# cvxpy/cvxpylayers

Hardware: AMD Instinct MI355X
Metric: forward+backward problems/sec, batch=4096 n=50 m=100 SOC (higher is better)
Workload: dtype f64; 1 GPU; config M: n=50 m=100 cones l=20 q=[10, 10, 10, 10, 10, 10, 10, 10] dense A (nnzA=5000), A,b,c batched, B=4096 per GPU, eps_abs=eps_rel=0.0001, max_iters=10000, Anderson acceleration (SCS default: acceleration_lookback=10, interval 10; engine: one-pair history); 4 distinct seeded batches resident in HBM, visited round-robin (warm-up and timed steps); step = plugin forward (layout pass + solve + sta; batch_per_gpu=4096, rotating_batches=4, parallelism=batch-shard x1

## Files before the change

### cvxpylayers_amd/csrc/ce_forward_v2.h

```cpp
#pragma once
#include "ce_common.h"
#include "ce_expcone.h"
#include "ce_wave_helpers.h"
#include "ce_psd_jacobi.h"
#include "ce_lds_fwd2.h"

#ifndef F2_MASK_MUL
#define F2_MASK_MUL 1
#endif
#if F2_MASK_MUL
#define F2_SEL(ix, expr) ((expr) * ((ix) >= 0 ? 1.0 : 0.0))
#else
#define F2_SEL(ix, expr) ((ix) >= 0 ? (expr) : 0.0)
#endif
#ifndef F2_SEG_PARTS
#define F2_SEG_PARTS 1
#endif
template <int CH, int TT, int PARTS_ = F2_SEG_PARTS, bool REDUCE = true>
__device__ __forceinline__ double seg_dot(const double (&tile)[TT], const double *vec) {
    const double2 *v2 = reinterpret_cast<const double2 *>(vec);
    double a0 = 0, a1 = 0;
    constexpr int NB = TT / 2, PARTS = NB > 8 ? PARTS_ : 1, H = (NB + PARTS - 1) / PARTS;
#pragma unroll
    for (int p = 0; p < PARTS; p++) {
#pragma unroll
        for (int k = p * H; k < (p + 1) * H && k < NB; k++) {
#ifdef F2_PROBE_HALFVEC
            const double2 v = v2[NB > 8 ? k % ((NB + 1) / 2) : k];
#else
            const double2 v = v2[k];
#endif
            a0 = fma(tile[2 * k], v.x, a0);
            a1 = fma(tile[2 * k + 1], v.y, a1);
        }
        if (p + 1 < PARTS) __builtin_amdgcn_sched_barrier(0);
    }
    if constexpr (REDUCE) return group_reduce<CH, false>(a0 + a1); else return a0 + a1;
}
template <int CH, int TT, bool REDUCE = true>
__device__ __forceinline__ double seg_dot_lds(const double *row, const double *vec) {
    const double2 *r2 = reinterpret_cast<const double2 *>(row), *v2 = reinterpret_cast<const double2 *>(vec);
    double a0 = 0, a1 = 0;
    constexpr int H = (TT / 2 + 1) / 2;
#pragma unroll
    for (int k = 0; k < H; k++) {
        const double2 r = r2[k], v = v2[k];
        a0 = fma(r.x, v.x, a0);
        a1 = fma(r.y, v.y, a1);
    }
    if constexpr (TT / 2 > 4) __builtin_amdgcn_sched_barrier(0);
#pragma unroll
    for (int k = H; k < TT / 2; k++) {
        const double2 r = r2[k], v = v2[k];
        a0 = fma(r.x, v.x, a0);
        a1 = fma(r.y, v.y, a1);
    }
    if constexpr (REDUCE) return group_reduce<CH, false>(a0 + a1); else return a0 + a1;
}

#ifndef F2_IDX_FENCE
#define F2_IDX_FENCE 8
#endif
template <int TT> constexpr int idx_stride = (TT + 3) & ~3;
template <int TT, class F>
__device__ __forceinline__ void for_each_idx(const int *__restrict__ base, int t, F &&f) {
    const int4 *ip = reinterpret_cast<const int4 *>(reinterpret_cast<const char *>(base) + (unsigned)t * (unsigned)(idx_stride<TT> * sizeof(int)));
#pragma unroll
    for (int c4 = 0; c4 < idx_stride<TT> / 4; c4++) {
        const int4 ix = ip[c4];
        if (4 * c4 + 0 < TT) f(std::integral_constant<int, 0>{}, 4 * c4 + 0, ix.x);
        if (4 * c4 + 1 < TT) f(std::integral_constant<int, 1>{}, 4 * c4 + 1, ix.y);
        if (4 * c4 + 2 < TT) f(std::integral_constant<int, 2>{}, 4 * c4 + 2, ix.z);
        if (4 * c4 + 3 < TT) f(std::integral_constant<int, 3>{}, 4 * c4 + 3, ix.w);
        if (c4 % F2_IDX_FENCE == F2_IDX_FENCE - 1) __builtin_amdgcn_sched_barrier(0);
    }
}

#ifndef F2_GATHER_CHUNK
#define F2_GATHER_CHUNK 14
#endif
template <int TT, class F>
__device__ __forceinline__ void gather_tile(const int *__restrict__ base, int t, const double *__restrict__ vals, F &&f) {
    const int4 *ip = reinterpret_cast<const int4 *>(reinterpret_cast<const char *>(base) + (unsigned)t * (unsigned)(idx_stride<TT> * sizeof(int)));
    int4 ix4[idx_stride<TT> / 4];
#pragma unroll
    for (int c4 = 0; c4 < idx_stride<TT> / 4; c4++) ix4[c4] = ip[c4];
    constexpr int CHK = F2_GATHER_CHUNK < TT ? F2_GATHER_CHUNK : TT;
#pragma unroll
    for (int k0 = 0; k0 < TT; k0 += CHK) {
        double raw[CHK];
#pragma unroll
        for (int u = 0; u < CHK; u++) {
            const int k = k0 + u < TT ? k0 + u : TT - 1;
            const int4 q = ix4[k >> 2];
            const int ix = (k & 3) == 0 ? q.x : ((k & 3) == 1 ? q.y : ((k & 3) == 2 ? q.z : q.w));
            raw[u] = vals[ix < 0 ? 0 : ix];
        }
        __builtin_amdgcn_sched_barrier(0);
#pragma unroll
        for (int u = 0; u < CHK; u++) {
            const int k = k0 + u;
            if (k < TT) {
                const int4 q = ix4[k >> 2];
                const int ix = (k & 3) == 0 ? q.x : ((k & 3) == 1 ? q.y : ((k & 3) == 2 ? q.z : q.w));
                const int msk = ~(ix >> 31);
                f(k, ix, __hiloint2double(__double2hiint(raw[u]) & msk, __double2loint(raw[u]) & msk));
            }
        }
        __builtin_amdgcn_sched_barrier(0);
    }
}

__device__ __forceinline__ void wave_lds_exchange() {
    __builtin_amdgcn_fence(__ATOMIC_RELEASE, "wavefront");
    __builtin_amdgcn_wave_barrier();
    __builtin_amdgcn_fence(__ATOMIC_ACQUIRE, "wavefront");
}

template <int CHT, int CHA, int CHG>
struct F2Co {
    int t, j1, c1, i2, c2, jg, cg;
    __device__ __forceinline__ static int thread_id(int wave) {
        int lane;
        asm volatile("v_mbcnt_lo_u32_b32 %0, -1, 0\n\tv_mbcnt_hi_u32_b32 %0, -1, %0" : "=v"(lane));
        return (wave << 6) + lane;
    }
    __device__ __forceinline__ explicit F2Co(int wave) {
        const unsigned u = (unsigned)thread_id(wave);
        t = (int)u;
        j1 = (int)(u / CHT); c1 = (int)(u % CHT); i2 = (int)(u / CHA); c2 = (int)(u % CHA); jg = (int)(u / CHG); cg = (int)(u % CHG);
    }
};

template <int K, int NWV>
__device__ __forceinline__ void block_reduce_w(double (&v)[K], unsigned maxmask, double *red, int wave) {
#pragma unroll
    for (int k = 0; k < K; k++) v[k] = ((maxmask >> k) & 1u) ? wave_reduce_dpp<true>(v[k]) : wave_reduce_dpp<false>(v[k]);
    if (__builtin_amdgcn_mbcnt_hi(~0u, __builtin_amdgcn_mbcnt_lo(~0u, 0u)) == 0) {
#pragma unroll
        for (int k = 0; k < K; k++) red[wave * K + k] = v[k];
    }
    __syncthreads();
#pragma unroll
    for (int k = 0; k < K; k++) {
        double t[NWV];
#pragma unroll
        for (int w = 0; w < NWV; w++) t[w] = red[w * K + k];
        double a = t[0];
#pragma unroll
        for (int w = 1; w < NWV; w++) a = ((maxmask >> k) & 1u) ? fmax(a, t[w]) : a + t[w];
        v[k] = a;
    }
    __syncthreads();
}

#ifdef CE_TIMING
#define F2_STAMP(i) do { __syncthreads(); if (threadIdx.x == 0) f2_tstamp[i] = __builtin_readcyclecounter(); } while (0)
#define F2_ACC(k) do { const long long t1_ = __builtin_readcyclecounter(); f2_tacc[k] += t1_ - f2_t0; f2_t0 = t1_; } while (0)
#define F2_EACC(k) do { const long long t1_ = __builtin_readcyclecounter(); f2_eacc[k] += t1_ - f2_t0; f2_t0 = t1_; } while (0)
#define F2_T0() do { f2_t0 = __builtin_readcyclecounter(); } while (0)
#else
#define F2_STAMP(i) do { } while (0)
#define F2_ACC(k) do { } while (0)
#define F2_EACC(k) do { } while (0)
#define F2_T0() do { } while (0)
#endif

#ifndef F2_WPS
#define F2_WPS 3
#endif
#ifndef F2_GJ_MFMA
#define F2_GJ_MFMA 1
#endif
template <int CHT, int T1, int CHA, int T2, int CHG, int TG, bool PSD = false, int NTH = 256, bool HASP = false, bool WL = false>
__global__ void __launch_bounds__(NTH, (NTH == 256 ? ((HASP || PSD) ? 2 : F2_WPS) : 2))
k_fwd2(DevT T, ce_settings S, const double *__restrict__ Avals, const double *__restrict__ qv, long sqk, long sqb,
       const int *__restrict__ idx_at, const int *__restrict__ idx_ar, const int *__restrict__ idx_b,
       double *__restrict__ xo, double *__restrict__ yo, double *__restrict__ so, int *__restrict__ iters_o,
       int *__restrict__ status_o, double *__restrict__ resid_o,
       const double *__restrict__ Pvals_g = nullptr, int nnzP = 0, const int *__restrict__ idx_p = nullptr,
       const int *__restrict__ row_perm = nullptr, const int *__restrict__ order = nullptr, int *__restrict__ iters2 = nullptr) {
    static_assert(!(WL && (PSD || HASP)), "wave-local cone exchange: plain cones only");
    constexpr int NT = NTH, NW = NTH / 64;
    using L = F2<CHT, T1, CHA, T2, CHG, TG, NW>;
    using Co = F2Co<CHT, CHA, CHG>;
    constexpr int MP = L::MP, NP = L::NP, VP = L::VP, OY = L::OY, OX = L::OX, OT = L::OT;
    extern __shared__ __attribute__((aligned(16))) double sm[];
    enum { SC_NB0 = 0, SC_NC0, SC_SIGMA, SC_SUMLOG, SC_RP, SC_RD, SC_GAP };
    double *const sc = sm + L::O_SC;
    double *const red = sm + L::O_RED;
    int *const socr = reinterpret_cast<int *>(sm + L::O_G);
    int *const socd = socr + MP;
    double *const Gm = sm + L::O_G + MP;

    const int tid = threadIdx.x, inst = (order && order[gridDim.x]) ? order[blockIdx.x] : blockIdx.x;
    const int wave = __builtin_amdgcn_readfirstlane(tid >> 6);
    const int n = T.n, m = T.m, l = n + m + 1, ldg = T.ldg, nq = T.nq, z = T.z;
    const int gsz = max(max(n * ldg, 4 * L::LDP), 16 * NP);
    const double *const vals = Avals + (size_t)inst * T.nnz_aug;

#ifdef CE_TIMING
    __shared__ long long f2_tstamp[24], f2_tstamp2[8];
    if (threadIdx.x < 24) f2_tstamp[threadIdx.x] = 0;
    long long f2_tacc[8] = {0, 0, 0, 0, 0, 0, 0, 0}, f2_t0 = 0;
    long long f2_eacc[8] = {0, 0, 0, 0, 0, 0, 0, 0};
#endif
    F2_STAMP(0);
    for (int i = tid; i < L::O_G; i += NT) sm[i] = 0.0;
    const double *const mtab = sm + L::O_MT;
    for (int i = tid; i < MP; i += NT) {
        int r0 = -1, d = 0;
        if (i < m) { const int c = T.rowcone[i]; if (c >= 0) { r0 = T.qoff[c]; d = T.qoff[c + 1] - r0; } }
        if constexpr (PSD) {
            for (int c = 0; c < T.ns; c++) if (i >= T.soff[c] && i < T.soff[c + 1]) { r0 = T.soff[c]; d = -(T.soff[c + 1] - r0); }
            if (i >= T.eoff && i < T.eoff + 3 * (T.nep + T.np)) { r0 = T.eoff + 3 * ((i - T.eoff) / 3); d = -3; }
        }
        socr[i] = r0; socd[i] = d;
    }
    __syncthreads();
    ce_math_table_init(sm + L::O_MT, tid);
    for (int i = tid; i < m; i += NT) { const int ix = idx_b[i]; const double v = vals[ix < 0 ? 0 : ix]; sm[L::O_BV + i] = ix >= 0 ? v : 0.0; sm[L::O_DV + i] = 1.0; }
    for (int j = tid; j < n; j += NT) { sm[L::O_CV + j] = qv[j * sqk + inst * sqb]; sm[L::O_EV + j] = 1.0; }
    __syncthreads();
    {
        double r[2] = {0, 0};
        for (int i = tid; i < m; i += NT) r[0] = fmax(r[0], fabs(sm[L::O_BV + i]));
        for (int j = tid; j < n; j += NT) r[1] = fmax(r[1], fabs(sm[L::O_CV + j]));
        block_reduce_w<2, NW>(r, 3u, red, wave);
        sc[SC_NB0] = r[0]; sc[SC_NC0] = r[1]; sc[SC_SIGMA] = 1.0; sc[9] = 0.0;
        sc[10] = sqrt((double)l); sc[11] = 1e10; sc[12] = 1e-300;
    }
    F2_STAMP(1);
    if (S.normalize) {
        const Co co(wave);
        const int j1 = co.j1, c1 = co.c1, i2 = co.i2, c2 = co.c2;
        const bool own1 = (c1 == 0) && (j1 < n), own2 = (c2 == 0) && (i2 < m);
        typedef float f2v __attribute__((ext_vector_type(2)));
        f2v atv[T1 / 2], arv[T2 / 2];
        float pf[HASP ? TG : 1];
        if constexpr (HASP) {
            const double *pv = Pvals_g + (size_t)inst * nnzP;
#pragma unroll
            for (int k = 0; k < TG; k++) { const int ix = idx_p[tid * idx_stride<TG> + k]; const double v = pv[ix < 0 ? 0 : ix]; pf[k] = ix >= 0 ? (float)v : 0.0f; }
        }
        float *const fPn = reinterpret_cast<float *>(sm + L::O_S3);
        gather_tile<T1>(idx_at, tid, vals, [&](int k, int ix, double v) { atv[k >> 1][k & 1] = ix >= 0 ? (float)(-v) : 0.0f; });
        gather_tile<T2>(idx_ar, tid, vals, [&](int k, int ix, double v) { arv[k >> 1][k & 1] = ix >= 0 ? (float)(-v) : 0.0f; });
        float *const fEt0 = reinterpret_cast<float *>(sm + L::O_S1), *const fEt1 = reinterpret_cast<float *>(sm + L::O_S2);
        float *const fDt0 = reinterpret_cast<float *>(sm + L::O_U + OY), *const fDt1 = reinterpret_cast<float *>(sm + L::O_UT + OY);
        float *const fRn = reinterpret_cast<float *>(sm + L::O_ZB + OY);
        auto clampf = [](float v) -> float { return v < (float)MIN_SCALE ? 1.0f : (v > (float)MAX_SCALE ? (float)MAX_SCALE : v); };
        double Eacc = 1.0, Dacc = 1.0;
        float ecum = 1.0f, dcum = 1.0f;
        const int blk_r0 = (i2 < m) ? socr[i2] : 0, blk_d = (i2 < m) ? abs(socd[i2]) : 0;
        F2_STAMP(14);
        F2_T0();
        for (int pass = 0; pass < NUM_RUIZ_PASSES + NUM_L2_PASSES; pass++) {
            const bool l2 = pass >= NUM_RUIZ_PASSES;
            float *const fEt = (pass & 1) ? fEt1 : fEt0;
            float *const fDt = (pass & 1) ? fDt1 : fDt0;
            float cn = 0, rn = 0;
            if (l2) {
#pragma unroll
                for (int k = 0; k < T1 / 2; k++) { cn = fmaf(atv[k].x, atv[k].x, cn); cn = fmaf(atv[k].y, atv[k].y, cn); }
#pragma unroll
                for (int k = 0; k < T2 / 2; k++) { rn = fmaf(arv[k].x, arv[k].x, rn); rn = fmaf(arv[k].y, arv[k].y, rn); }
                cn = ecum * sqrtf(group_reduce_f<CHT, false>(cn)); rn = dcum * sqrtf(group_reduce_f<CHA, false>(rn));
            } else {
                float c0 = 0, c1_ = 0, r0 = 0, r1 = 0;
#pragma unroll
                for (int k = 0; k < T1 / 2; k += 2) { c0 = fmaxf(fmaxf(c0, fabsf(atv[k].x)), fabsf(atv[k].y)); if (k + 1 < T1 / 2) c1_ = fmaxf(fmaxf(c1_, fabsf(atv[k + 1].x)), fabsf(atv[k + 1].y)); }
#pragma unroll
                for (int k = 0; k < T2 / 2; k += 2) { r0 = fmaxf(fmaxf(r0, fabsf(arv[k].x)), fabsf(arv[k].y)); if (k + 1 < T2 / 2) r1 = fmaxf(fmaxf(r1, fabsf(arv[k + 1].x)), fabsf(arv[k + 1].y)); }
                cn = ecum * group_reduce_f<CHT, true>(fmaxf(c0, c1_)); rn = dcum * group_reduce_f<CHA, true>(fmaxf(r0, r1));
            }
            if constexpr (HASP) {
                const Co cop(wave);
                float pn = 0;
                if (l2) {
#pragma unroll
                    for (int k = 0; k < TG; k++) pn = fmaf(pf[k], pf[k], pn);
                    pn = group_reduce_f<CHG, false>(pn);
                } else {
#pragma unroll
                    for (int k = 0; k < TG; k++) pn = fmaxf(pn, fabsf(pf[k]));
                    pn = group_reduce_f<CHG, true>(pn);
                }
                if (cop.cg == 0 && cop.jg < n) fPn[cop.jg] = pn;
            } else {
                if (own1) fEt[j1] = __builtin_amdgcn_rsqf(clampf(cn));
            }
            if (own2) fRn[i2] = rn;
            F2_EACC(0);
            if constexpr (WL) wave_lds_exchange(); else __syncthreads();
            if constexpr (HASP) {
                if (own1) { const float pn = fPn[j1]; fEt[j1] = __builtin_amdgcn_rsqf(clampf(l2 ? sqrtf(cn * cn + pn) : fmaxf(cn, pn))); }
            }
            constexpr int NEQ = (12 + CHA - 1) / CHA;
            float ssh = 0;
            if (blk_d > 1 && blk_d <= 12) {
                const int off = (int)__umul24((unsigned)c2, (unsigned)NEQ);
                const float *fr = fRn + blk_r0 + off;
                const int lim = blk_d - off;
                float v[NEQ];
#pragma unroll
                for (int u = 0; u < NEQ; u++) v[u] = fr[u];
#pragma unroll
                for (int u = 0; u < NEQ; u++) ssh += (u < lim) ? v[u] : 0.0f;
            }
            ssh = group_reduce_f<CHA, false>(ssh);
            if (own2) {
                float a = rn;
                const int r0 = blk_r0, d = blk_d;
                if (d > 1) {
                    float s0 = ssh, s1 = 0;
                    if (d <= 12) {
                    } else {
                        int i = 0;
                        for (; i + 1 < d; i += 2) { s0 += fRn[r0 + i]; s1 += fRn[r0 + i + 1]; }
                        if (i < d) s0 += fRn[r0 + i];
                    }
                    a = (s0 + s1) * __builtin_amdgcn_rcpf((float)d);
                }
                fDt[i2] = __builtin_amdgcn_rsqf(clampf(a));
            }
            F2_EACC(1);
            __syncthreads();
            F2_EACC(2);
            {
                const float ej = fEt[j1 < NP ? j1 : 0];
                const float di = fDt[i2 < MP ? i2 : 0];
                const f2v *d2 = reinterpret_cast<const f2v *>(fDt + T1 * c1);
                const f2v *e2 = reinterpret_cast<const f2v *>(fEt + T2 * c2);
                f2v dd[T1 / 2], ee[T2 / 2];
#pragma unroll
                for (int k = 0; k < T1 / 2; k++) dd[k] = d2[k];
#pragma unroll
                for (int k = 0; k < T2 / 2; k++) ee[k] = e2[k];
                __builtin_amdgcn_sched_barrier(0);
#pragma unroll
                for (int k = 0; k < T1 / 2; k++) atv[k] *= dd[k];
#pragma unroll
                for (int k = 0; k < T2 / 2; k++) arv[k] *= ee[k];
                ecum *= ej; dcum *= di;
                if constexpr (HASP) {
                    const Co cop(wave);
                    const float eg = fEt[cop.jg < NP ? cop.jg : 0];
                    const float2 *g2 = reinterpret_cast<const float2 *>(fEt + TG * cop.cg);
#pragma unroll
                    for (int k = 0; k < TG / 2; k++) { const float2 ee = g2[k]; pf[2 * k] *= eg * ee.x; pf[2 * k + 1] *= eg * ee.y; }
                }
                Eacc *= (double)ej; Dacc *= (double)di;
            }
            F2_EACC(3);
        }
        F2_STAMP(15);
        if (own1) sm[L::O_EV + j1] = Eacc;
        if (own2) sm[L::O_DV + i2] = Dacc;
        __syncthreads();
        double r[2] = {0, 0};
        for (int i = tid; i < m; i += NT) { const double v = sm[L::O_BV + i] * sm[L::O_DV + i]; sm[L::O_BV + i] = v; r[0] = fmax(r[0], fabs(v)); }
        for (int j = tid; j < n; j += NT) { const double v = sm[L::O_CV + j] * sm[L::O_EV + j]; sm[L::O_CV + j] = v; r[1] = fmax(r[1], fabs(v)); }
        block_reduce_w<2, NW>(r, 3u, red, wave);
        const double sigma = 1.0 / clamp_scale(fmax(r[0], r[1]));
        sc[SC_SIGMA] = sigma;
        for (int i = tid; i < m; i += NT) sm[L::O_BV + i] *= sigma;
        for (int j = tid; j < n; j += NT) sm[L::O_CV + j] *= sigma;
        for (int i = tid; i < VP; i += NT) { sm[L::O_U + i] = 0.0; sm[L::O_UT + i] = 0.0; sm[L::O_ZB + i] = 0.0; }
        for (int i = tid; i < NP; i += NT) { sm[L::O_S1 + i] = 0.0; sm[L::O_S2 + i] = 0.0; }
        __syncthreads();
    }

    F2_STAMP(2);
    double scale = S.scale, hg = 0, inv_den = 0;
    const double rho_x = S.rho_x, rtau = TAU_FACTOR, alpha = S.alpha;
    auto dyv = [&](int i) -> double { return (i < z) ? ZERO_CONE_FACTOR * scale : scale; };

    double at[T1], ar[T2];
    auto materialize_at = [&](const Co &co) {
        const double ej = sm[L::O_EV + (co.j1 < NP ? co.j1 : 0)];
        const double *dv = sm + L::O_DV + T1 * co.c1;
        gather_tile<T1>(idx_at, co.t, vals, [&](int k, int ix, double v) { at[k] = F2_SEL(ix, -v * (dv[k] * ej)); });
    };
    auto materialize_ar = [&](const Co &co) {
        const double di = sm[L::O_DV + (co.i2 < MP ? co.i2 : 0)];
        const double *evs = sm + L::O_EV + T2 * co.c2;
        gather_tile<T2>(idx_ar, co.t, vals, [&](int k, int ix, double v) { ar[k] = F2_SEL(ix, -v * (di * evs[k])); });
    };
    double gPg = 0;
    double *const PgV = Gm + gsz;
    auto materialize_p = [&](const Co &co, double (&pg)[TG]) {
        const double *pv = Pvals_g + (size_t)inst * nnzP;
        const double ej = sm[L::O_EV + (co.jg < NP ? co.jg : 0)];
        const double *evs = sm + L::O_EV + TG * co.cg;
        gather_tile<TG>(idx_p, co.t, pv, [&](int k, int ix, double v) { pg[k] = F2_SEL(ix, v * (ej * evs[k])); });
    };
    auto load_phi_tile = [&](const Co &co) {
        if (co.j1 == n) {
#pragma unroll
            for (int k = 0; k < T1; k++) at[k] = sm[L::O_PHI + OY + T1 * co.c1 + k];
        } else if (co.j1 == n + 1) {
#pragma unroll
            for (int k = 0; k < T1; k++) at[k] = (T1 * co.c1 + k < n) ? sm[L::O_PHI + OX + T1 * co.c1 + k] : 0.0;
        }
    };

    double g_scale = 0.0;
    auto refactor = [&]() {
        F2_STAMP(7);
        const Co co(wave);
        const int tid = co.t;
        const int j1 = co.j1, c1 = co.c1, i2 = co.i2, c2 = co.c2, jg = co.jg, cg = co.cg;
        const bool own1 = (c1 == 0) && (j1 < n), own2 = (c2 == 0) && (i2 < m), owng = (cg == 0) && (jg < n);
        double sreg[TG];
#pragma unroll
        for (int s = 0; s < TG; s++) sreg[s] = 0.0;
        bool fast = false, g_in_lds = false;
        if constexpr (!HASP && TG <= 14) {
            if (T.f2_neumann && g_scale > 0.0) {
                const double f = uniform_d(scale / g_scale), delta = uniform_d(rho_x * (1.0 - f) / f);
                double r[1] = {0};
                if (jg < n) {
                    const double2 *src = reinterpret_cast<const double2 *>(Gm + jg * ldg + TG * cg);
#pragma unroll
                    for (int s2 = 0; s2 < TG / 2; s2++) { const double2 v = src[s2]; r[0] = fma(v.x, v.x, fma(v.y, v.y, r[0])); }
                }
                block_reduce_w<1, NW>(r, 0u, red, wave);
                const int ex = __builtin_amdgcn_readfirstlane((__double2hiint(fabs(delta) * sqrt(r[0])) >> 20) & 0x7ff) - 1023;
                const int K = ex < -17 ? 2 : (ex < -13 ? 3 : (ex < -10 ? 4 : (ex < -7 ? 7 : 0)));
                if (K > 0) {
                    fast = true;
                    double greg[TG];
                    if (jg < n) {
                        const double2 *src = reinterpret_cast<const double2 *>(Gm + jg * ldg + TG * cg);
#pragma unroll
                        for (int s2 = 0; s2 < TG / 2; s2++) { const double2 v = src[s2]; sreg[2 * s2] = v.x; sreg[2 * s2 + 1] = v.y; }
                    }
#pragma unroll
                    for (int s = 0; s < TG; s++) greg[s] = sreg[s];
                    const int lane_base = (threadIdx.x & 63) & ~(CHG - 1);
                    for (int it = 0; it < K; it++) {
                        double zz[TG];
#pragma unroll
                        for (int s = 0; s < TG; s++) zz[s] = 0.0;
                        int goff = TG * cg;
                        asm volatile("" : "+v"(goff));
#pragma unroll
                        for (int q = 0; q < CHG; q++) {
                            const int src_lane = (lane_base + q) << 2;
#pragma unroll
                            for (int s = 0; s < TG; s++) {
                                const int kcol = TG * q + s;
                                const int lo = __builtin_amdgcn_ds_bpermute(src_lane, __double2loint(sreg[s])), hi = __builtin_amdgcn_ds_bpermute(src_lane, __double2hiint(sreg[s]));
                                const double yk = __hiloint2double(hi, lo);
                                if (kcol < n) {
                                    const double2 *gr = reinterpret_cast<const double2 *>(Gm + goff);
                                    goff += ldg;
#pragma unroll
                                    for (int s2 = 0; s2 < TG / 2; s2++) { const double2 v = gr[s2]; zz[2 * s2] = fma(yk, v.x, zz[2 * s2]); zz[2 * s2 + 1] = fma(yk, v.y, zz[2 * s2 + 1]); }
                                }
                            }
                        }
#pragma unroll
                        for (int s = 0; s < TG; s++) sreg[s] = fma(-delta, zz[s], greg[s]);
                    }
                    const double rf = 1.0 / f;
#pragma unroll
                    for (int s = 0; s < TG; s++) sreg[s] = (jg < n) ? sreg[s] * rf : 0.0;
                    __syncthreads();
                }
            }
        }
        if (!fast) {
        materialize_ar(co);
#pragma unroll
        for (int s = 0; s < TG; s++) sreg[s] = 0.0;
        {
            constexpr int NTILE = L::NTILE, LDP = L::LDP;
            typedef double v4d __attribute__((ext_vector_type(4)));
            v4d acc[NTILE];
#pragma unroll
            for (int J = 0; J < NTILE; J++) acc[J] = v4d{0.0, 0.0, 0.0, 0.0};
            const int PR = (gsz / LDP) & ~3;
            const int lane = tid & 63, lg = lane >> 4, lc = lane & 15;
            for (int p0 = 0; p0 < m; p0 += PR) {
                const int p1 = min(m, p0 + PR), rows4 = (p1 - p0 + 3) & ~3;
                if (i2 >= p0 && i2 < p1) {
                    double2 *dst = reinterpret_cast<double2 *>(Gm + (i2 - p0) * LDP + T2 * c2);
#pragma unroll
                    for (int k = 0; k < T2 / 2; k++) dst[k] = make_double2(ar[2 * k], ar[2 * k + 1]);
                }
                for (int i = tid; i < (p1 - p0) * (LDP - L::NPa); i += NT) Gm[(i / (LDP - L::NPa)) * LDP + L::NPa + i % (LDP - L::NPa)] = 0.0;
                for (int i = tid; i < (rows4 - (p1 - p0)) * LDP; i += NT) Gm[(p1 - p0) * LDP + i] = 0.0;
                __syncthreads();
                if (wave < NTILE) {
                    const double *prow = Gm + lg * LDP + lc;
                    for (int i0 = 0; i0 < rows4; i0 += 4, prow += 4 * LDP) {
                        const double a = prow[16 * wave] * dyv(p0 + i0 + lg);
#pragma unroll
                        for (int J = 0; J < NTILE; J++) acc[J] = __builtin_amdgcn_mfma_f64_16x16x4f64(a, prow[16 * J], acc[J], 0, 0, 0);
                    }
                }
                __syncthreads();
            }
            if constexpr (F2_GJ_MFMA && !HASP) {
                static_assert(8 * LDP <= 16 * NP, "two R buffers of four rows fit the exchange region");
                constexpr int MAXB = 4 * NTILE;
                const int NB = (n + 3) >> 2;
                if (wave < NTILE) {
                    static_for<NTILE>([&](auto Jc) {
                        constexpr int J = decltype(Jc)::value;
                        if (wave == J) {
#pragma unroll
                            for (int r = 0; r < 4; r++) { const int row = 16 * J + lg + 4 * r; if (lc == lg + 4 * r) acc[J][r] += (row < n ? rho_x : 1.0); }
                        }
                    });
                    if (wave == 0) {
#pragma unroll
                        for (int J = 0; J < NTILE; J++) Gm[lg * LDP + 16 * J + lc] = acc[J][0];
                    }
                }
                __syncthreads();
                F2_STAMP(8);
                F2_T0();
                static_for<MAXB>([&](auto bc) {
                    constexpr int b = decltype(bc)::value, k0 = 4 * b, wo = k0 / 16, r0 = (k0 % 16) / 4, c0 = k0 % 16;
                    constexpr int k1 = k0 + 4, wn = (k1 / 16) % NTILE, r1 = (k1 % 16) / 4;
                    if (b < NB) {
                        const double *Rb = Gm + (b & 1) * (4 * LDP);
                        double *Rn = Gm + ((b + 1) & 1) * (4 * LDP);
                        if (wave < NTILE) {
                            double Bop[NTILE], Cop[4], a[4][4];
#pragma unroll
                            for (int J = 0; J < NTILE; J++) Bop[J] = Rb[lg * LDP + 16 * J + lc];
                            {
                                int coff = 16 * wave + lc;
                                asm volatile("" : "+v"(coff));
#pragma unroll
                                for (int pq = 0; pq < 4; pq++) Cop[pq] = Rb[pq * LDP + coff];
                            }
#pragma unroll
                            for (int q = 0; q < 4; q++) {
                                const double2 v0 = *reinterpret_cast<const double2 *>(Rb + q * LDP + k0), v1 = *reinterpret_cast<const double2 *>(Rb + q * LDP + k0 + 2);
                                a[q][0] = v0.x; a[q][1] = v0.y; a[q][2] = v1.x; a[q][3] = v1.y;
                            }
                            __builtin_amdgcn_sched_barrier(0);
                            double e[4];
#pragma unroll
                            for (int k = 0; k < 4; k++) e[k] = (lg == k) ? 1.0 : 0.0;
                            double pinv[4];
#pragma unroll
                            for (int k = 0; k < 4; k++) {
                                const double pv = a[k][k];
                                double pi_ = __builtin_amdgcn_rcp(pv);
                                pi_ = fma(fma(-pv, pi_, 1.0), pi_, pi_);
                                pi_ = fma(fma(-pv, pi_, 1.0), pi_, pi_);
                                pinv[k] = pi_;
#pragma unroll
                                for (int i = k + 1; i < 4; i++) {
                                    const double lm = a[i][k] * pi_;
#pragma unroll
                                    for (int j = k + 1; j < 4; j++) a[i][j] = fma(-lm, a[k][j], a[i][j]);
                                    e[i] = fma(-lm, e[k], e[i]);
                                }
                            }
                            double xs[4];
                            xs[3] = e[3] * pinv[3];
                            xs[2] = fma(-a[2][3], xs[3], e[2]) * pinv[2];
                            xs[1] = fma(-a[1][3], xs[3], fma(-a[1][2], xs[2], e[1])) * pinv[1];
                            xs[0] = fma(-a[0][3], xs[3], fma(-a[0][2], xs[2], fma(-a[0][1], xs[1], e[0]))) * pinv[0];
                            F2_EACC(4);
                            double wsel = -(Cop[0] * xs[0] + Cop[1] * xs[1] + Cop[2] * xs[2] + Cop[3] * xs[3]);
                            const int mr = lc - c0;
                            const bool kcol = mr >= 0 && mr < 4;
                            const double nk = kcol ? 0.0 : 1.0;
                            if (wave == wo) {
                                double psel = 0.0;
#pragma unroll
                                for (int k = 0; k < 4; k++) psel = fma(xs[k], (mr == k) ? 1.0 : 0.0, psel);
                                wsel = fma(wsel, nk, psel);
#pragma unroll
                                for (int J = 0; J < NTILE; J++) acc[J][r0] = 0.0;
                            }
#pragma unroll
                            for (int r = 0; r < 4; r++) acc[wo][r] *= nk;
                            Bop[wo] = fma(Bop[wo], nk, (kcol && mr == lg) ? -1.0 : 0.0);
                            F2_EACC(5);
#pragma unroll
                            for (int J = 0; J < NTILE; J++) acc[J] = __builtin_amdgcn_mfma_f64_16x16x4f64(wsel, Bop[J], acc[J], 0, 0, 0);
                            F2_EACC(6);
                            if (b + 1 < NB && wave == wn) {
#pragma unroll
                                for (int J = 0; J < NTILE; J++) Rn[lg * LDP + 16 * J + lc] = acc[J][r1];
                            }
                        }
                        __syncthreads();
                        F2_EACC(7);
                    }
                });
                F2_STAMP(9);
                if (wave < NTILE) {
#pragma unroll
                    for (int J = 0; J < NTILE; J++)
#pragma unroll
                        for (int r = 0; r < 4; r++) {
                            const int row = 16 * wave + lg + 4 * r, col = 16 * J + lc;
                            if (row < n && col < L::NPg) Gm[row * ldg + col] = 0.0 - acc[J][r];
                        }
                }
                g_in_lds = true;
            } else {
                if (wave < NTILE) {
#pragma unroll
                    for (int J = 0; J < NTILE; J++)
#pragma unroll
                        for (int r = 0; r < 4; r++) {
                            const int row = 16 * wave + lg + 4 * r, col = 16 * J + lc;
                            if (row < n && col < L::NPg) Gm[row * ldg + col] = acc[J][r] + (row == col ? rho_x : 0.0);
                        }
                }
                __syncthreads();
                if (jg < n) {
                    const double2 *src = reinterpret_cast<const double2 *>(Gm + jg * ldg + TG * cg);
#pragma unroll
                    for (int s = 0; s < TG / 2; s++) { const double2 v = src[s]; sreg[2 * s] = v.x; sreg[2 * s + 1] = v.y; }
                }
                __syncthreads();
                if constexpr (HASP) {
                    double pg[TG];
                    materialize_p(co, pg);
#pragma unroll
                    for (int s = 0; s < TG; s++) if (jg < n) sreg[s] += pg[s];
                }
            }
        }
        if (!g_in_lds) {
        F2_STAMP(8);
        constexpr int NBLK = (TG + 3) / 4;
        auto rbuf = [&](int b) -> double * { return Gm + b * (8 * NP); };
        auto cbuf = [&](int b) -> double * { return Gm + b * (8 * NP) + 4 * NP; };
        auto publish = [&](auto blk_c, int cgn, int bufn) {
            constexpr int kk0 = 4 * decltype(blk_c)::value;
            const int k0 = TG * cgn + kk0;
            if (jg < n && cg == cgn) {
                double2 *dst = reinterpret_cast<double2 *>(cbuf(bufn) + 4 * jg);
                dst[0] = make_double2(sreg[kk0], sreg[kk0 + 1]);
                if constexpr (kk0 + 3 < TG) dst[1] = make_double2(sreg[kk0 + 2], sreg[kk0 + 3]);
            }
            if (jg >= k0 && jg < k0 + (TG - kk0 < 4 ? TG - kk0 : 4) && jg < n) {
                double2 *dst = reinterpret_cast<double2 *>(rbuf(bufn) + (jg - k0) * NP + TG * cg);
#pragma unroll
                for (int s = 0; s < TG / 2; s++) dst[s] = make_double2(sreg[2 * s], sreg[2 * s + 1]);
            }
        };
        for (int i = tid; i < 16 * NP; i += NT) Gm[i] = 0.0;
        __syncthreads();
        int cnt = 0;
        publish(std::integral_constant<int, 0>{}, 0, 0);
        __syncthreads();
        F2_T0();
        static_for<NBLK>([&](auto blk_c) {
            constexpr int blk = decltype(blk_c)::value, kk0 = 4 * blk;
            constexpr int NBS = (TG - kk0) < 4 ? (TG - kk0) : 4;
            const int nv = (kk0 < n) ? (n - 1 - kk0) / TG + 1 : 0;
            const int nvn = (kk0 + 4 < TG && kk0 + 4 < n) ? 1 : 0;
            for (int cgk = 0; cgk < nv; cgk++) {
                const int k0 = TG * cgk + kk0, buf = cnt & 1;
                const int nbv = min(NBS, n - k0);
                const double *rb = rbuf(buf), *cb = cbuf(buf);
                if (jg < n) {
                    double a[4][4];
#pragma unroll
                    for (int q = 0; q < 4; q++) {
                        const double2 v0 = *reinterpret_cast<const double2 *>(rb + q * NP + k0), v1 = *reinterpret_cast<const double2 *>(rb + q * NP + k0 + 2);
                        a[q][0] = v0.x; a[q][1] = v0.y; a[q][2] = v1.x; a[q][3] = v1.y;
                    }
                    if (nbv < 4) {
#pragma unroll
                        for (int q = 0; q < 4; q++)
#pragma unroll
                            for (int q2 = 0; q2 < 4; q2++) if (!(q < nbv && q2 < nbv)) a[q][q2] = (q == q2 ? 1.0 : 0.0);
                    }
                    bool bad = false;
#pragma unroll
                    for (int p = 0; p < 4; p++) {
                        const double pv = a[p][p];
                        bad = bad || !(pv > 0);
                        double pinv = __builtin_amdgcn_rcp(pv);
                        pinv = fma(fma(-pv, pinv, 1.0), pinv, pinv);
                        pinv = fma(fma(-pv, pinv, 1.0), pinv, pinv);
#pragma unroll
                        for (int j = 0; j < 4; j++) if (j != p) a[p][j] *= pinv;
#pragma unroll
                        for (int i = 0; i < 4; i++) if (i != p) {
                            const double f = a[i][p];
#pragma unroll
                            for (int j = 0; j < 4; j++) if (j != p) a[i][j] = fma(-f, a[p][j], a[i][j]);
                            a[i][p] = -f * pinv;
                        }
                        a[p][p] = pinv;
                    }
                    F2_EACC(4);
                    if constexpr (HASP) { if (bad && jg == k0 && cg == 0) sc[7] = 1.0; }
                    const double2 c01 = reinterpret_cast<const double2 *>(cb + 4 * jg)[0];
                    double2 c23 = make_double2(0.0, 0.0);
                    if constexpr (NBS > 2) c23 = reinterpret_cast<const double2 *>(cb + 4 * jg)[1];
                    const int qrow = jg - k0;
                    const bool prow_thread = (qrow >= 0 && qrow < NBS);
                    double w[4];
#pragma unroll
                    for (int q = 0; q < 4; q++) {
                        const double wc = -(c01.x * a[0][q] + c01.y * a[1][q] + c23.x * a[2][q] + c23.y * a[3][q]);
                        const double wp = qrow == 0 ? a[0][q] : (qrow == 1 ? a[1][q] : (qrow == 2 ? a[2][q] : a[3][q]));
                        w[q] = prow_thread ? wp : wc;
                    }
                    F2_EACC(5);
                    const double2 *r0 = reinterpret_cast<const double2 *>(rb + TG * cg), *r1 = reinterpret_cast<const double2 *>(rb + NP + TG * cg),
                                  *r2 = reinterpret_cast<const double2 *>(rb + 2 * NP + TG * cg), *r3 = reinterpret_cast<const double2 *>(rb + 3 * NP + TG * cg);
#pragma unroll
                    for (int s2 = 0; s2 < TG / 2; s2++) {
                        const double2 v0 = r0[s2], v1 = r1[s2], v2 = r2[s2], v3 = r3[s2];
                        const double bx = prow_thread ? 0.0 : sreg[2 * s2], by = prow_thread ? 0.0 : sreg[2 * s2 + 1];
                        sreg[2 * s2] = fma(w[3], v3.x, fma(w[2], v2.x, fma(w[1], v1.x, fma(w[0], v0.x, bx))));
                        sreg[2 * s2 + 1] = fma(w[3], v3.y, fma(w[2], v2.y, fma(w[1], v1.y, fma(w[0], v0.y, by))));
                    }
                    if (cg == cgk) {
#pragma unroll
                        for (int q = 0; q < NBS; q++) sreg[kk0 + q] = w[q];
                    }
                }
                F2_EACC(6);
                if (cgk + 1 < nv) publish(std::integral_constant<int, blk>{}, cgk + 1, buf ^ 1);
                else if (nvn) publish(std::integral_constant<int, (blk + 1 < NBLK ? blk + 1 : blk)>{}, 0, buf ^ 1);
                cnt++;
                __syncthreads();
                F2_EACC(7);
            }
        });
        F2_STAMP(9);
        }
        }
        g_scale = uniform_d(scale);
        if constexpr (HASP) { if (sc[7] != 0.0) return; }
        if (!g_in_lds && jg < n) {
            double2 *dst = reinterpret_cast<double2 *>(Gm + jg * ldg + TG * cg);
#pragma unroll
            for (int s = 0; s < TG / 2; s++) dst[s] = make_double2(sreg[2 * s], sreg[2 * s + 1]);
        }
        for (int i = tid; i < NP; i += NT) { sm[L::O_S1 + i] = 0.0; sm[L::O_S2 + i] = 0.0; sm[L::O_S3 + i] = 0.0; sm[L::O_S4 + i] = 0.0; }
        for (int i = tid; i < m; i += NT) sm[L::O_ZB + OY + i] = dyv(i) * sm[L::O_BV + i];
        __syncthreads();
        materialize_at(co);
        {
            const double a = seg_dot<CHT, T1>(at, sm + L::O_ZB + OY + T1 * c1);
            if (own1) { const double cj = sm[L::O_CV + j1]; sm[L::O_S1 + j1] = cj - a; sm[L::O_S2 + j1] = cj + a; }
        }
        __syncthreads();
        F2_STAMP(11);
        {
            const double *grow = Gm + (jg < n ? jg : 0) * ldg + TG * cg;
            const double gx = seg_dot_lds<CHG, TG>(grow, sm + L::O_S1 + TG * cg), gk = seg_dot_lds<CHG, TG>(grow, sm + L::O_S2 + TG * cg);
            if (owng) { sm[L::O_GV + OX + jg] = gx; sm[L::O_PX + jg] = gk; }
        }
        __syncthreads();
        F2_STAMP(12);
        if constexpr (HASP) {
            double pg[TG];
            materialize_p(co, pg);
            const double a = seg_dot<CHG, TG>(pg, sm + L::O_GV + OX + TG * cg);
            if (owng) PgV[jg] = a;
            __syncthreads();
            double rg[1] = {tid < n ? sm[L::O_GV + OX + tid] * PgV[tid] : 0.0};
            block_reduce_w<1, NW>(rg, 0u, red, wave);
            gPg = uniform_d(rg[0]);
        }
        materialize_ar(co);
        double r[1] = {0};
        {
            const double agx = seg_dot<CHA, T2>(ar, sm + L::O_GV + OX + T2 * c2);
            __builtin_amdgcn_sched_barrier(0);
            const double agk = seg_dot<CHA, T2>(ar, sm + L::O_PX + T2 * c2);
            __builtin_amdgcn_sched_barrier(0);
            if (own2) {
                const double bi = sm[L::O_BV + i2];
                const double gy = dyv(i2) * (agx + bi);
                sm[L::O_GV + OY + i2] = gy; r[0] += bi * gy;
                sm[L::O_PHI + OY + i2] = bi - agk;
            }
            if (tid < n) { r[0] += sm[L::O_CV + tid] * sm[L::O_GV + OX + tid]; sm[L::O_PHI + OX + tid] = rho_x * sm[L::O_PX + tid]; }
        }
        F2_STAMP(13);
        block_reduce_w<1, NW>(r, 0u, red, wave);
        hg = uniform_d(r[0]);
        inv_den = uniform_d(1.0 / (rtau + hg));
        load_phi_tile(co);
        for (int i = tid; i < NP; i += NT) { sm[L::O_S1 + i] = 0.0; sm[L::O_S2 + i] = 0.0; sm[L::O_PX + i] = 0.0; }
        for (int i = tid; i < m; i += NT) sm[L::O_ZB + OY + i] = 0.0;
        __syncthreads();
        F2_STAMP(10);
    };

    if (threadIdx.x == 0) sm[L::O_W + OT] = 1.0;
    if (S.warm_start) {
        const double sg = sc[SC_SIGMA];
        const int inst_ = inst;
        double wx = 0, wy = 0; bool bad = false;
        const int e = threadIdx.x;
        if (e < n) { wx = sg * xo[(size_t)inst_ * n + e] / sm[L::O_EV + e]; bad = !(fabs(wx) < 1e300); }
        for (int i = e; i < m; i += NT) {
            const double dvi = sm[L::O_DV + i];
            const int io = WL ? row_perm[i] : i;
            const double v = sg * yo[(size_t)inst_ * m + io] / dvi + sg * dvi * so[(size_t)inst_ * m + io] * dyv(i);
            bad = bad || !(fabs(v) < 1e300);
        }
        double rb[1] = {bad ? 1.0 : 0.0};
        block_reduce_w<1, NW>(rb, 1u, red, wave);
        if (rb[0] == 0.0) {
            if (e < n) sm[L::O_W + OX + e] = wx;
            for (int i = e; i < m; i += NT) {
                const double dvi = sm[L::O_DV + i];
                const int io = WL ? row_perm[i] : i;
                sm[L::O_W + OY + i] = sg * yo[(size_t)inst_ * m + io] / dvi + sg * dvi * so[(size_t)inst_ * m + io] * dyv(i);
            }
        }
    }
    __syncthreads();

    int status = 0, iter = 0, last_scale_iter = 0, n_log = 0;
    int aa_ph = 0, chk_ph = 0;
    auto next_iter = [&]() { iter++; aa_ph = (aa_ph + 1 >= S.acceleration_interval) ? 0 : aa_ph + 1; chk_ph = (chk_ph + 1 == CONVERGED_INTERVAL) ? 0 : chk_ph + 1; };
    bool aa_on = S.acceleration_lookback > 0;
    const int aa_int = S.acceleration_interval;
    double *const aaWP = Gm + gsz + (PSD ? ((T.ns > 0 ? 2 * T.maxs * T.maxs + 2 * T.maxs + 8 : 0) + T.nep + T.np) : 0) + (HASP ? NP : 0);
    double *const aaXP = aaWP + VP, *const aaFP = aaXP + VP, *const aaFS = aaFP + VP, *const aaXS = aaFS + VP;
    int aa_iter = 0; bool aa_pending = false, aa_stale = false;
    const bool big_soc = T.maxq > SOC_SMALL;
    bool resume = false;

    auto project_e = [&](int e, int ve) -> double {
        double ue = sm[L::O_ZB + ve];
        const int soc_d = (e < m) ? socd[e] : 0;
        if (soc_d > 1 && !big_soc) {
            const int soc_r0 = socr[e];
            const double *zc = sm + L::O_ZB + OY + soc_r0;
            const double t0 = zc[0];
            double q0 = 0, q1 = 0;
            if (soc_d <= 13) {
                double zv[12];
#pragma unroll
                for (int u = 0; u < 12; u++) zv[u] = zc[1 + u];
#pragma unroll
                for (int u = 0; u < 12; u += 2) {
                    const double z0 = (1 + u < soc_d) ? zv[u] : 0.0, z1 = (2 + u < soc_d) ? zv[u + 1] : 0.0;
                    q0 = fma(z0, z0, q0); q1 = fma(z1, z1, q1);
                }
            } else {
                for (int k = 1; k < soc_d; k += 4) {
                    const double z0 = zc[k], z1 = (k + 1 < soc_d) ? zc[k + 1] : 0.0, z2 = (k + 2 < soc_d) ? zc[k + 2] : 0.0, z3 = (k + 3 < soc_d) ? zc[k + 3] : 0.0;
                    q0 = fma(z0, z0, q0); q1 = fma(z1, z1, q1); q0 = fma(z2, z2, q0); q1 = fma(z3, z3, q1);
                }
            }
            const double q = q0 + q1;
            double nz = 0, rinv = 0;
            if (q > 0) sqrt_rsqrt(q, nz, rinv);
            if (nz <= t0) {  }
            else if (nz <= -t0) ue = 0.0;
            else { const double c0 = 0.5 * (t0 + nz); ue = (e == soc_r0) ? c0 : ue * (c0 * rinv); }
        } else if (soc_d == 1) ue = fmax(ue, 0.0);
        return ue;
    };
    auto slot_of = [&](int e) -> int { return (e < m) ? OY + e : (e < m + n ? OX + (e - m) : OT); };

    if constexpr (PSD) {
        double *expR0 = Gm + gsz + (T.ns > 0 ? 2 * T.maxs * T.maxs + 2 * T.maxs + 8 : 0);
        for (int c = tid; c < T.nep + T.np; c += NT) expR0[c] = 0.0;
    }
    for (bool done = false; !done;) {
    refactor();
    if constexpr (HASP) { if (sc[7] != 0.0) { status = -4; break; } }
    F2_STAMP(3);
    if (resume) {
        const int e = Co::thread_id(wave);
        if (e < l) { const int ve = slot_of(e); sm[L::O_W + ve] += alpha * (sm[L::O_U + ve] - sm[L::O_UT + ve]); }
        __syncthreads();
        resume = false; next_iter();
    }
    for (;;) {
        if (iter >= S.max_iters) { done = true; break; }
        const Co co(wave);
        const int j1 = co.j1, c1 = co.c1, i2 = co.i2, c2 = co.c2, jg = co.jg, cg = co.cg;
        const bool own1 = (c1 == 0) && (j1 < n), own2 = (c2 == 0) && (i2 < m), owng = (cg == 0) && (jg < n);
        const int e = co.t;
        const int ve = slot_of(e);
        const bool ev = e < l;
        const bool check = chk_ph == 0;
        const bool last = iter + 1 >= S.max_iters;
        F2_ACC(6);
        if (aa_on) {
            if (aa_pending) {
                const double dd = ev ? aaWP[ve] - sm[L::O_W + ve] : 0.0;
                double r[1] = {dd * dd};
                block_reduce_w<1, NW>(r, 0u, red, wave);
                if (!(uniform_d(r[0]) <= sc[8])) {
                    if (ev) { sm[L::O_W + ve] = aaFS[ve]; aaWP[ve] = aaXS[ve]; }
                    aa_iter = 0;
                    if (Co::thread_id(wave) == 0) sc[9] += 1.0;
                    __syncthreads();
                    if (uniform_d(sc[9]) >= AA_MAX_REJECT) aa_on = false;
                }
                aa_pending = false;
            }
            if (aa_on && iter > 0 && aa_ph == 0 && !aa_stale) {
                const double xv = ev ? aaWP[ve] : 0.0, fv = ev ? sm[L::O_W + ve] : 0.0, gv = xv - fv;
                if (aa_iter > 0) {
                    const double xp = ev ? aaXP[ve] : 0.0, fp = ev ? aaFP[ve] : 0.0;
                    const double sv = xv - xp, yv = gv - (xp - fp), dv = fv - fp;
                    double r[5] = {sv * sv, yv * yv, sv * yv, sv * gv, gv * gv};
                    block_reduce_w<5, NW>(r, 0u, red, wave);
                    double s01 = 0, ri01 = 0;
                    { const double q01 = r[0] * r[1]; if (q01 > 0) sqrt_rsqrt(q01, s01, ri01); }
                    const double mm = uniform_d(r[2] + 1e-8 * s01);
                    double mi = __builtin_amdgcn_rcp(mm);
                    mi = fma(fma(-mm, mi, 1.0), mi, mi);
                    mi = fma(fma(-mm, mi, 1.0), mi, mi);
                    const double gam = uniform_d(r[3] * mi);
                    if (ev) { aaXP[ve] = xv; aaFP[ve] = fv; }
                    int o11 = 11; asm volatile("" : "+s"(o11));
                    if (fabs(mm) > sc[o11 + 1]  && fabs(gam) < sc[o11] ) {
                        if (ev) { aaFS[ve] = fv; aaXS[ve] = xv; sm[L::O_W + ve] = fv - gam * dv; }
                        if (Co::thread_id(wave) == 0) sc[8] = r[4];
                        aa_pending = true;
                    } else aa_iter = 0;
                } else if (ev) { aaXP[ve] = xv; aaFP[ve] = fv; }
                aa_iter++;
                __syncthreads();
            }
        }
        if (check && iter > 0) {
            const double we = ev ? sm[L::O_W + ve] : 0.0;
            double r[1] = {we * we};
            block_reduce_w<1, NW>(r, 0u, red, wave);
            const double nw = uniform_d(sqrt(r[0]));
            if (nw > 0 && ev) {
                int o10 = 10; asm volatile("" : "+s"(o10));
                const double fsc = sc[o10] / nw;
                sm[L::O_W + ve] = we * fsc;
                if (aa_on) {
                    aaXP[ve] *= fsc; aaFP[ve] *= fsc; aaFS[ve] *= fsc; aaXS[ve] *= fsc;
                    if (e == 0) sc[8] *= fsc * fsc;
                }
            }
            __syncthreads();
        }
        if (aa_on && (aa_pending || aa_ph + 1 == aa_int)) { aa_stale = false; if (ev) aaWP[ve] = sm[L::O_W + ve]; }
        F2_ACC(0);
        {
            const double *wvec = sm + L::O_W + ((j1 == n + 1 && T1 * c1 < n) ? OX : OY) + T1 * c1;
            const double a = seg_dot<CHT, T1>(at, wvec);
            if (own1) sm[L::O_TV + j1] = rho_x * sm[L::O_W + OX + j1] - a;
            else if (c1 == 0 && j1 <= n + 1) sm[L::O_WP + (j1 - n)] = a;
        }
        F2_ACC(1);
        __syncthreads();
        F2_ACC(2);
        {
            const double a = seg_dot_lds<CHG, TG>(Gm + __mul24(jg < n ? jg : 0, ldg) + TG * cg, sm + L::O_TV + TG * cg);
            if (owng) sm[L::O_PX + jg] = a;
            if (WL && Co::thread_id(wave) == 0) sm[L::O_WP + 2] = sm[L::O_W + OT];
        }
        F2_ACC(3);
        __syncthreads();
        F2_ACC(2);
        if constexpr (WL) {
            const int ee = OY + i2;
            const bool upd = !check && !last;
            double we = 0, gve = 0;
            int cd = 0, soc_r0 = 0;
            if (own2) { we = sm[L::O_W + ee]; gve = sm[L::O_GV + ee]; }
            if (i2 < m) { cd = socd[i2]; soc_r0 = socr[i2]; }
            const double wp0 = sm[L::O_WP], wp1 = sm[L::O_WP + 1], wp2 = sm[L::O_WP + 2];
            const double q = seg_dot<CHA, T2>(ar, sm + L::O_PX + T2 * c2);
            __builtin_amdgcn_sched_barrier(0);
            const double tau_t = (rtau * wp2 + wp0 + wp1) * inv_den;
            double ute = 0, ze = 0;
            if (own2) {
                const double py = we + dyv(i2) * q;
                ute = py - tau_t * gve;
                ze = 2 * ute - we;
                if (cd == 1 && ze < 0) ze = 0;
                sm[L::O_UT + ee] = ute; sm[L::O_ZB + ee] = ze;
            }
            F2_ACC(4);
            wave_lds_exchange();
            constexpr int NE = (12 + CHA - 1) / CHA;
            double qsh = 0;
            if (cd > 1 && cd <= 13) {
                const int off = (int)__umul24((unsigned)c2, (unsigned)NE);
                const double *zc = sm + L::O_ZB + OY + soc_r0 + 1 + off;
                const int lim = cd - 1 - off;
                double zv[NE];
#pragma unroll
                for (int u = 0; u < NE; u++) zv[u] = zc[u];
                double q0 = 0, q1 = 0;
#pragma unroll
                for (int u = 0; u < NE; u++) {
                    const double zz = (u < lim) ? zv[u] : 0.0;
                    if (u & 1) q1 = fma(zz, zz, q1); else q0 = fma(zz, zz, q0);
                }
                qsh = q0 + q1;
            }
            qsh = group_reduce<CHA, false>(qsh);
            if (own2) {
                double ue = ze;
                if (cd > 1) {
                    const double *zc = sm + L::O_ZB + OY + soc_r0;
                    const double t0 = zc[0];
                    double q0 = qsh, q1 = 0;
                    if (cd <= 13) {
                    } else {
                        for (int k = 1; k < cd; k += 4) {
                            const double z0 = zc[k], z1 = (k + 1 < cd) ? zc[k + 1] : 0.0, z2 = (k + 2 < cd) ? zc[k + 2] : 0.0, z3 = (k + 3 < cd) ? zc[k + 3] : 0.0;
                            q0 = fma(z0, z0, q0); q1 = fma(z1, z1, q1); q0 = fma(z2, z2, q0); q1 = fma(z3, z3, q1);
                        }
                    }
                    const double qq = q0 + q1;
                    double nz = 0, rinv = 0;
                    if (qq > 0) sqrt_rsqrt(qq, nz, rinv);
                    if (nz <= t0) {  }
                    else if (nz <= -t0) ue = 0.0;
                    else { const double c0 = 0.5 * (t0 + nz); ue = (i2 == soc_r0) ? c0 : ue * (c0 * rinv); }
                }
                sm[L::O_U + ee] = ue;
                if (upd) sm[L::O_W + ee] = we + alpha * (ue - ute);
            }
            if (e < n) {
                const int ex = OX + e;
                const double wx = sm[L::O_W + ex];
                const double utx = sm[L::O_PX + e] - tau_t * sm[L::O_GV + ex];
                const double ux = 2 * utx - wx;
                sm[L::O_UT + ex] = utx; sm[L::O_U + ex] = ux;
                if (upd) sm[L::O_W + ex] = wx + alpha * (ux - utx);
            }
            if (e == NT - 1) {
                const double wt = sm[L::O_W + OT];
                const double ut = fmax(0.0, 2 * tau_t - wt);
                sm[L::O_UT + OT] = tau_t; sm[L::O_U + OT] = ut;
                if (upd) sm[L::O_W + OT] = wt + alpha * (ut - tau_t);
            }
            F2_ACC(5);
            __syncthreads();
            F2_ACC(2);
            if (upd) { next_iter(); continue; }
        } else {
        {
            const double wt0 = sm[L::O_W + OT], wp0 = sm[L::O_WP], wp1 = sm[L::O_WP + 1];
            const double q = seg_dot<CHA, T2>(ar, sm + L::O_PX + T2 * c2);
            __builtin_amdgcn_sched_barrier(0);
            double tau_t = (rtau * wt0 + wp0 + wp1) * inv_den;
            if constexpr (HASP) {
                double r3[3] = {0, 0, 0};
                if (own2) { const double py = sm[L::O_W + OY + i2] + dyv(i2) * q; r3[0] = q * py; }
                if (e < n) { const double px = sm[L::O_PX + e]; r3[1] = px * (sm[L::O_W + OX + e] - px); r3[2] = px * PgV[e]; }
                block_reduce_w<3, NW>(r3, 0u, red, wave);
                const double pPp = rho_x * r3[1] - r3[0];
                const double qa = rtau + hg - gPg, qb = -(rtau * sm[L::O_W + OT] + sm[L::O_WP] + sm[L::O_WP + 1]) + 2 * r3[2];
                tau_t = uniform_d((-qb + sqrt(fmax(qb * qb + 4 * qa * fmax(pPp, 0.0), 0.0))) / (2 * qa));
            }
            if (own2) {
                const int ee = OY + i2;
                const double we = sm[L::O_W + ee];
                const double py = we + dyv(i2) * q;
                const double ute = py - tau_t * sm[L::O_GV + ee];
                double ze = 2 * ute - we;
                if (i2 >= z && i2 < z + T.l && ze < 0) ze = 0;
                sm[L::O_UT + ee] = ute; sm[L::O_ZB + ee] = ze;
            }
            if (e < n) {
                const int ee = OX + e;
                const double ute = sm[L::O_PX + e] - tau_t * sm[L::O_GV + ee];
// ... 185 lines not shown
```

Before: 1.979 million problems/s.

## Build transposed A tile via LDS transpose and keep ar registers across phases

In the normalize phase, the transposed tile (atv) is no longer gathered a second time from global memory. It is built by writing the already-gathered row tile (arv) into LDS as floats and reading it back column-wise. A KEEP_AR mode also keeps the equilibrated ar registers alive from the factorization phase, so the later materialize_ar gather is skipped when the non-fast path ran. The gather-chunk size for these one-shot gathers is raised to the full tile. The intent is to cut redundant global gathers at the cost of extra LDS traffic, barriers and register pressure.

New measurement: 1.969 million problems/s (median of 2 runs). No clear change (-0.5%).

```diff
diff --git a/cvxpylayers_amd/csrc/ce_forward_v2.h b/cvxpylayers_amd/csrc/ce_forward_v2.h
--- a/cvxpylayers_amd/csrc/ce_forward_v2.h
+++ b/cvxpylayers_amd/csrc/ce_forward_v2.h
@@ -79,13 +79,15 @@
 #ifndef F2_GATHER_CHUNK
 #define F2_GATHER_CHUNK 14
 #endif
-template <int TT, class F>
-__device__ __forceinline__ void gather_tile(const int *__restrict__ base, int t, const double *__restrict__ vals, F &&f) {
+template <int TT>
+__device__ __forceinline__ void load_idx_row(const int *__restrict__ base, int t, int4 (&ix4)[idx_stride<TT> / 4]) {
     const int4 *ip = reinterpret_cast<const int4 *>(reinterpret_cast<const char *>(base) + (unsigned)t * (unsigned)(idx_stride<TT> * sizeof(int)));
-    int4 ix4[idx_stride<TT> / 4];
 #pragma unroll
     for (int c4 = 0; c4 < idx_stride<TT> / 4; c4++) ix4[c4] = ip[c4];
-    constexpr int CHK = F2_GATHER_CHUNK < TT ? F2_GATHER_CHUNK : TT;
+}
+template <int TT, int CHUNK, class F>
+__device__ __forceinline__ void gather_vals(const int4 (&ix4)[idx_stride<TT> / 4], const double *__restrict__ vals, F &&f) {
+    constexpr int CHK = CHUNK < TT ? CHUNK : TT;
 #pragma unroll
     for (int k0 = 0; k0 < TT; k0 += CHK) {
         double raw[CHK];
@@ -109,6 +111,12 @@
         }
         __builtin_amdgcn_sched_barrier(0);
     }
+}
+template <int TT, int CHUNK = F2_GATHER_CHUNK, class F>
+__device__ __forceinline__ void gather_tile(const int *__restrict__ base, int t, const double *__restrict__ vals, F &&f) {
+    int4 ix4[idx_stride<TT> / 4];
+    load_idx_row<TT>(base, t, ix4);
+    gather_vals<TT, CHUNK>(ix4, vals, f);
 }
 
 __device__ __forceinline__ void wave_lds_exchange() {
@@ -171,6 +179,12 @@
 #endif
 #ifndef F2_GJ_MFMA
 #define F2_GJ_MFMA 1
+#endif
+#ifndef F2_ATV_LDS
+#define F2_ATV_LDS 1
+#endif
+#ifndef F2_KEEP_AR
+#define F2_KEEP_AR 1
 #endif
 template <int CHT, int T1, int CHA, int T2, int CHG, int TG, bool PSD = false, int NTH = 256, bool HASP = false, bool WL = false>
 __global__ void __launch_bounds__(NTH, (NTH == 256 ? ((HASP || PSD) ? 2 : F2_WPS) : 2))
@@ -244,8 +258,36 @@
             for (int k = 0; k < TG; k++) { const int ix = idx_p[tid * idx_stride<TG> + k]; const double v = pv[ix < 0 ? 0 : ix]; pf[k] = ix >= 0 ? (float)v : 0.0f; }
         }
         float *const fPn = reinterpret_cast<float *>(sm + L::O_S3);
-        gather_tile<T1>(idx_at, tid, vals, [&](int k, int ix, double v) { atv[k >> 1][k & 1] = ix >= 0 ? (float)(-v) : 0.0f; });
-        gather_tile<T2>(idx_ar, tid, vals, [&](int k, int ix, double v) { arv[k >> 1][k & 1] = ix >= 0 ? (float)(-v) : 0.0f; });
+        gather_tile<T2, T2>(idx_ar, tid, vals, [&](int k, int ix, double v) { arv[k >> 1][k & 1] = ix >= 0 ? (float)(-v) : 0.0f; });
+#if F2_ATV_LDS
+        {
+            constexpr int LDF = L::NPa + 2;
+            float *const Tf = reinterpret_cast<float *>(Gm);
+            const int PRF = (2 * gsz) / LDF;
+#pragma unroll
+            for (int k = 0; k < T1 / 2; k++) atv[k] = f2v{0.0f, 0.0f};
+            for (int p0 = 0; p0 < m; p0 += PRF) {
+                const int np = min(m, p0 + PRF) - p0;
+                if (p0) __syncthreads();
+                if (i2 >= p0 && i2 < p0 + np) {
+                    f2v *dst = reinterpret_cast<f2v *>(Tf + (i2 - p0) * LDF + T2 * c2);
+#pragma unroll
+                    for (int k = 0; k < T2 / 2; k++) dst[k] = arv[k];
+                }
+                __syncthreads();
+                const int rb = (int)__umul24((unsigned)c1, (unsigned)T1) - p0;
+                const float *pcol = Tf + (j1 < n ? j1 : 0);
+#pragma unroll
+                for (int k = 0; k < T1; k++) {
+                    const bool in = (unsigned)(rb + k) < (unsigned)np && j1 < n;
+                    const float v = pcol[(in ? rb + k : 0) * LDF];
+                    atv[k >> 1][k & 1] = in ? v : atv[k >> 1][k & 1];
+                }
+            }
+        }
+#else
+        gather_tile<T1, T1>(idx_at, tid, vals, [&](int k, int ix, double v) { atv[k >> 1][k & 1] = ix >= 0 ? (float)(-v) : 0.0f; });
+#endif
         float *const fEt0 = reinterpret_cast<float *>(sm + L::O_S1), *const fEt1 = reinterpret_cast<float *>(sm + L::O_S2);
         float *const fDt0 = reinterpret_cast<float *>(sm + L::O_U + OY), *const fDt1 = reinterpret_cast<float *>(sm + L::O_UT + OY);
         float *const fRn = reinterpret_cast<float *>(sm + L::O_ZB + OY);
@@ -382,10 +424,10 @@
         const double *dv = sm + L::O_DV + T1 * co.c1;
         gather_tile<T1>(idx_at, co.t, vals, [&](int k, int ix, double v) { at[k] = F2_SEL(ix, -v * (dv[k] * ej)); });
     };
-    auto materialize_ar = [&](const Co &co) {
+    auto materialize_ar = [&](const Co &co, auto chunk_c) {
         const double di = sm[L::O_DV + (co.i2 < MP ? co.i2 : 0)];
         const double *evs = sm + L::O_EV + T2 * co.c2;
-        gather_tile<T2>(idx_ar, co.t, vals, [&](int k, int ix, double v) { ar[k] = F2_SEL(ix, -v * (di * evs[k])); });
+        gather_tile<T2, decltype(chunk_c)::value>(idx_ar, co.t, vals, [&](int k, int ix, double v) { ar[k] = F2_SEL(ix, -v * (di * evs[k])); });
     };
     double gPg = 0;
     double *const PgV = Gm + gsz;
@@ -416,6 +458,11 @@
 #pragma unroll
         for (int s = 0; s < TG; s++) sreg[s] = 0.0;
         bool fast = false, g_in_lds = false;
+        constexpr bool KEEP_AR = F2_KEEP_AR && F2_GJ_MFMA && !HASP && (WL || PSD || NTH != 256 || T1 + T2 <= 32);
+        if constexpr (KEEP_AR) {
+#pragma unroll
+            for (int k = 0; k < T2; k++) ar[k] = 0.0;
+        }
         if constexpr (!HASP && TG <= 14) {
             if (T.f2_neumann && g_scale > 0.0) {
                 const double f = uniform_d(scale / g_scale), delta = uniform_d(rho_x * (1.0 - f) / f);
@@ -472,7 +519,7 @@
             }
         }
         if (!fast) {
-        materialize_ar(co);
+        materialize_ar(co, std::integral_constant<int, T2>{});
 #pragma unroll
         for (int s = 0; s < TG; s++) sreg[s] = 0.0;
         {
@@ -774,7 +821,7 @@
             block_reduce_w<1, NW>(rg, 0u, red, wave);
             gPg = uniform_d(rg[0]);
         }
-        materialize_ar(co);
+        if (!KEEP_AR || fast) materialize_ar(co, std::integral_constant<int, F2_GATHER_CHUNK>{});
         double r[1] = {0};
         {
             const double agx = seg_dot<CHA, T2>(ar, sm + L::O_GV + OX + T2 * c2);
```
